# zju-pi/diff-sampler

Measured on AMD Instinct MI355X. Metric: images/sec (whole node) at NFE=10, EDM CIFAR-10, higher is better.
Workload: dtype fp32; 1 GPU; EDM CIFAR-10 32x32 SongUNet (55.7M params), DPM-Solver++(2M) logSNR NFE=10, batch 256/GPU; launch=eager

## Files before the change

diff_sampler_amd/csrc/conv3x3_wino.hip:

```cpp
#include <type_traits>

#include "igemm_common.h"

namespace igemm {
namespace {

typedef float f32x2 __attribute__((ext_vector_type(2)));

constexpr int WV_NO_NORM = 2, WV_NO_HALO = 4, WV_NO_DMA = 8, WV_NO_EPI = 16;
constexpr int WINO_K = 8;
constexpr int WINO_POS = 2 * 64 * 4;
constexpr int WINO_IMG = 16 * WINO_POS;
constexpr int WINO_NSH = 4;
constexpr int WINO_EPI_LD = 36;

#define DS_WINO_WAIT_VM0() do { __builtin_amdgcn_s_waitcnt(0x0F70); asm volatile("" ::: "memory"); } while (0)
#define DS_WINO_WAIT_VM(n) do { __builtin_amdgcn_s_waitcnt(0x0F70 | (n)); asm volatile("" ::: "memory"); } while (0)

template <int VAR, int NORM, int NSL>
__global__ void __launch_bounds__(256, 1) conv3x3_wino_kernel(const KParams p) {
    extern __shared__ __attribute__((aligned(16))) float smem[];
    float* Us = smem;
    float* Vs = smem + 2 * WINO_IMG;
    float* Hs = smem + 4 * WINO_IMG;
// ... 566 lines not shown
    };

    f32x16 acc[16];
#pragma unroll
    for (int q = 0; q < 16; ++q)
#pragma unroll
        for (int r = 0; r < 16; ++r) acc[q][r] = 0.f;
    const int a_off = ((lane >> 5) * 32 + (lane & 31)) * 4;

#define DS_WINO_I(n) std::integral_constant<int, (n)>{}
#define DS_WINO_EACH4(F) F(0) F(1) F(2) F(3)
#define DS_WINO_EACH12(F) F(0) F(1) F(2) F(3) F(4) F(5) F(6) F(7) F(8) F(9) F(10) F(11)
#define DS_WINO_EACH16(F, b) F((b) + 0) F((b) + 1) F((b) + 2) F((b) + 3) F((b) + 4) F((b) + 5) F((b) + 6) F((b) + 7)                \
                             F((b) + 8) F((b) + 9) F((b) + 10) F((b) + 11) F((b) + 12) F((b) + 13) F((b) + 14) F((b) + 15)
#define DS_WINO_LOADS(R, sl)                                                                                                           \
    halo_load1(R, DS_WINO_I(0)); halo_load1(R, DS_WINO_I(1)); halo_load1(R, DS_WINO_I(2));                                             \
    coef_load1(R, sl, DS_WINO_I(0)); coef_load1(R, sl, DS_WINO_I(1)); coef_load1(R, sl, DS_WINO_I(2));

    halo_src(0);
    DS_WINO_LOADS(hreg, 0)
    {
        HaloRegs hreg1;
        const int s1 = min(1, nslabs - 1);
        halo_src(s1);
        DS_WINO_LOADS(hreg1, s1)
#define DS_WINO_F(i) b_load1(u_src, DS_WINO_I(0), DS_WINO_I(i));
        DS_WINO_EACH4(DS_WINO_F)
#undef DS_WINO_F
        DS_RACE_SKEW(wave);
#define DS_WINO_CHAIN1(c) halo_chain(hreg, Hs, DS_WINO_I(c), DS_WINO_I(0)); halo_chain(hreg, Hs, DS_WINO_I(c), DS_WINO_I(1));          \
                          halo_chain(hreg, Hs, DS_WINO_I(c), DS_WINO_I(2));
        DS_WINO_EACH12(DS_WINO_CHAIN1)
#undef DS_WINO_CHAIN1
        DS_RACE_SKEW(wave);
#define DS_WINO_CHAIN1(c) halo_chain(hreg1, Hs + h_buf, DS_WINO_I(c), DS_WINO_I(0)); halo_chain(hreg1, Hs + h_buf, DS_WINO_I(c), DS_WINO_I(1)); \
                          halo_chain(hreg1, Hs + h_buf, DS_WINO_I(c), DS_WINO_I(2));
        DS_WINO_EACH12(DS_WINO_CHAIN1)
#undef DS_WINO_CHAIN1
    }
    {
        const int s2 = min(2, nslabs - 1);
        halo_src(s2);
        DS_WINO_LOADS(hreg, s2)
    }
    __syncthreads();
#define DS_WINO_TR1(i) tr_read1(Hs, DS_WINO_I(i));
    DS_WINO_EACH12(DS_WINO_TR1)
#undef DS_WINO_TR1
    DS_RACE_SKEW(wave);
    tr_write(Vs);
    DS_WINO_WAIT_VM0();
    __syncthreads();

    int s = 0;
    do {
        const int par = s & 1;
        const float* vb = Vs + par * WN_IMG;
        float* vbn = Vs + (par ^ 1) * WN_IMG;
        float* hb = Hs + par * h_buf;
        const float* hbn = Hs + (par ^ 1) * h_buf;
        const int s1 = min(s + 1, nslabs - 1), s3 = min(s + 3, nslabs - 1);
        const float* uc = u_src + (size_t)s * WINO_IMG;
        const float* un = u_src + (size_t)s1 * WINO_IMG;
        auto a_read = [&](auto G, auto I) {
            constexpr int g = decltype(G)::value, i = decltype(I)::value;
            fa[g & 1][i] = *reinterpret_cast<const f32x4*>(vb + (g * 4 + i) * WN_POS + a_off);
        };
#define DS_WINO_TR1(i) tr_read1(hbn, DS_WINO_I(i));
        DS_WINO_EACH12(DS_WINO_TR1)
#undef DS_WINO_TR1
        DS_RACE_SKEW(wave);
#define DS_WINO_CHAIN1(c) halo_chain(hreg, hb, DS_WINO_I(c), DS_WINO_I(0)); halo_chain(hreg, hb, DS_WINO_I(c), DS_WINO_I(1));          \
                          halo_chain(hreg, hb, DS_WINO_I(c), DS_WINO_I(2));
        DS_WINO_EACH12(DS_WINO_CHAIN1)
#undef DS_WINO_CHAIN1
        halo_src(s3);
        DS_RACE_SKEW(wave);
        tr_write(vbn);
        auto fill = [&](auto K) {
            constexpr int k = decltype(K)::value, g = k >> 4, q = k & 15;
            if constexpr (q < 4) {
                if constexpr (g < 3) b_load1(uc, DS_WINO_I(g + 1), DS_WINO_I(q));
                else b_load1(un, DS_WINO_I(0), DS_WINO_I(q));
            } else if constexpr (k < 7) {
                halo_load1(hreg, DS_WINO_I(k - 4));
            } else if constexpr (k < 10) {
                coef_load1(hreg, s3, DS_WINO_I(k - 7));
            } else if constexpr (q >= 10 && q < 14 && g < 3) {
                a_read(DS_WINO_I(g + 1), DS_WINO_I(q - 10));
            }
        };
#define DS_WINO_STEP(k)                                                                                                                \
        acc[((k) >> 4) * 4 + ((k) & 3)] = __builtin_amdgcn_mfma_f32_32x32x2f32(fa[((k) >> 4) & 1][(k) & 3][((k) >> 2) & 3],            \
                                                                               fb[((k) >> 4) & 1][(k) & 3][((k) >> 2) & 3],            \
                                                                               acc[((k) >> 4) * 4 + ((k) & 3)], 0, 0, 0);              \
        fill(DS_WINO_I(k));                                                                                                            \
        __builtin_amdgcn_sched_barrier(0);
#define DS_WINO_F(i) a_read(DS_WINO_I(0), DS_WINO_I(i));
        DS_WINO_EACH4(DS_WINO_F)
#undef DS_WINO_F
        __builtin_amdgcn_sched_barrier(0);
        DS_WINO_EACH16(DS_WINO_STEP, 0)
        DS_WINO_EACH16(DS_WINO_STEP, 16)
        DS_WINO_EACH16(DS_WINO_STEP, 32)
        DS_WINO_EACH16(DS_WINO_STEP, 48)
#undef DS_WINO_STEP
        __syncthreads();
    } while (++s < nslabs);
#undef DS_WINO_LOADS

    f32x16 Y[4];
#pragma unroll
    for (int a = 0; a < 2; ++a) {
        f32x16 t[4];
#pragma unroll
        for (int j = 0; j < 4; ++j) t[j] = a == 0 ? acc[j] + acc[4 + j] + acc[8 + j] : acc[4 + j] - acc[8 + j] - acc[12 + j];
        Y[a * 2 + 0] = t[0] + t[1] + t[2];
        Y[a * 2 + 1] = t[1] - t[2] - t[3];
    }

    const int nextra = (p.ec0 + p.ec1) / 32;
    if (nextra > 0) {
        const float* wsk = p.b + (size_t)(p.N / 64) * nslabs * WINO_IMG + (size_t)(2 * nt + (wave >> 1)) * nextra * 2048;
        const int e_chunk = tid & 7;
        int e_lds[4];
#pragma unroll
        for (int j = 0; j < 4; ++j) {
            const int lp = (tid >> 3) + 32 * j;
            const int yl = lp / p.W, x = lp - yl * p.W;
            const int ph = (yl & 1) * 2 + (x & 1), t = (yl >> 1) * Wt + (x >> 1);
            e_lds[j] = (((ph * 4 + (e_chunk >> 1)) * 2 + (e_chunk & 1)) * 32 + (t ^ e_chunk)) * 4;
        }
        int ea_off[4];
#pragma unroll
        for (int g = 0; g < 4; ++g) ea_off[g] = ((lane >> 5) * 32 + ((lane & 31) ^ (2 * g + (lane >> 5)))) * 4;
        const unsigned e_t0 = (unsigned)((tid >> 3) * p.elda0 + e_chunk * 4), e_t1 = (unsigned)((tid >> 3) * p.elda1 + e_chunk * 4);
        const float* e_src = nullptr;
        unsigned e_off = 0;
        int e_step = 0;
        auto e_sel = [&](int es) {
            const int c = es * 32;
            const bool first = c < p.ec0;
            const int ld = first ? p.elda0 : p.elda1;
            e_src = (first ? p.e0 + c : p.e1 + (c - p.ec0)) + (size_t)m0 * ld;
            e_step = 32 * ld;
            e_off = first ? e_t0 : e_t1;
        };
        auto e_load1 = [&](f32x4* dst, auto J) {
            constexpr int j = decltype(J)::value;
            dst[j] = *reinterpret_cast<const f32x4*>(e_src + (size_t)(j * e_step) + e_off);
        };
        f32x4 ga[2][4], gb[2];
        auto w_load1 = [&](int es, auto G) {
            constexpr int g = decltype(G)::value;
            const char* ws = reinterpret_cast<const char*>(wsk + (size_t)es * 2048 + g * WINO_POS);
            asm volatile("" : "+s"(ws));
            asm volatile("" : "+v"(b_lane));
            gb[g & 1] = *(gf4_t)(ws + b_lane);
        };

        f32x4 ereg[4];
        {
            f32x4 ereg0[4];
            w_load1(0, DS_WINO_I(0));
            e_sel(0);
#define DS_WINO_F(j) e_load1(ereg0, DS_WINO_I(j));
            DS_WINO_EACH4(DS_WINO_F)
#undef DS_WINO_F
            e_sel(min(1, nextra - 1));
#define DS_WINO_F(j) e_load1(ereg, DS_WINO_I(j));
            DS_WINO_EACH4(DS_WINO_F)
#undef DS_WINO_F
            DS_RACE_SKEW(wave);
#pragma unroll
            for (int j = 0; j < 4; ++j) *reinterpret_cast<f32x4*>(Vs + e_lds[j]) = ereg0[j];
        }
        __syncthreads();

        int es = 0;
        do {
            const float* vb = smem + (es & 1) * WN_IMG;
            float* vn = smem + ((es + 1) & 1) * WN_IMG;
            const int es1 = min(es + 1, nextra - 1);
            e_sel(min(es + 2, nextra - 1));
            auto a_read = [&](auto G, auto I) {
                constexpr int g = decltype(G)::value, i = decltype(I)::value;
                ga[g & 1][i] = *reinterpret_cast<const f32x4*>(vb + (i * 4 + g) * WN_POS + ea_off[g]);
            };
            auto fill = [&](auto K) {
                constexpr int k = decltype(K)::value, g = k >> 4, q = k & 15;
                if constexpr (q == 0) {
                    if constexpr (g < 3) w_load1(es, DS_WINO_I(g + 1));
                    else w_load1(es1, DS_WINO_I(0));
                } else if constexpr (q < 5) {
                    if constexpr (g < 3) a_read(DS_WINO_I(g + 1), DS_WINO_I(q - 1));
                } else if constexpr (k < 9) {
                    if constexpr (k == 5) DS_RACE_SKEW(wave);
                    *reinterpret_cast<f32x4*>(vn + e_lds[k - 5]) = ereg[k - 5];
                } else if constexpr (k < 13) {
                    e_load1(ereg, DS_WINO_I(k - 9));
                }
            };
#define DS_WINO_STEP(k)                                                                                                                \
            Y[(k) & 3] = __builtin_amdgcn_mfma_f32_32x32x2f32(ga[((k) >> 4) & 1][(k) & 3][((k) >> 2) & 3], gb[((k) >> 4) & 1][((k) >> 2) & 3], \
                                                              Y[(k) & 3], 0, 0, 0);                                                    \
            fill(DS_WINO_I(k));                                                                                                        \
            __builtin_amdgcn_sched_barrier(0);
#define DS_WINO_F(i) a_read(DS_WINO_I(0), DS_WINO_I(i));
            DS_WINO_EACH4(DS_WINO_F)
#undef DS_WINO_F
            __builtin_amdgcn_sched_barrier(0);
            DS_WINO_EACH16(DS_WINO_STEP, 0)
            DS_WINO_EACH16(DS_WINO_STEP, 16)
            DS_WINO_EACH16(DS_WINO_STEP, 32)
            DS_WINO_EACH16(DS_WINO_STEP, 48)
#undef DS_WINO_STEP
            __syncthreads();
        } while (++es < nextra);
    }
#undef DS_WINO_EACH16
#undef DS_WINO_EACH12
#undef DS_WINO_EACH4
#undef DS_WINO_I

    float* stage = smem + wave * 32 * WINO_EPI_LD;
    const int c4 = (lane & 7) * 4;
    const int col = n0 + wave * 32 + c4;
    f32x4 cb = {0.f, 0.f, 0.f, 0.f}, cvu = {0.f, 0.f, 0.f, 0.f};
    if (p.colbias) cb = *reinterpret_cast<const f32x4*>(p.colbias + col);
    if (p.cbias) cvu = *reinterpret_cast<const f32x4*>(p.cbias + (size_t)(p.cbias_bcast ? 0 : img0) * p.cbias_ld + col);
    const float acc_scale = __builtin_bit_cast(float, __builtin_amdgcn_readfirstlane(__builtin_bit_cast(int, p.acc_scale)));
    const float scale = __builtin_bit_cast(float, __builtin_amdgcn_readfirstlane(__builtin_bit_cast(int, p.scale)));
    int e_row[4];
#pragma unroll
    for (int pass = 0; pass < 4; ++pass) {
        const int tl = pass * 8 + (lane >> 3);
        const int ty = tl / Wt, tx = tl - ty * Wt;
        e_row[pass] = m0 + 2 * ty * p.W + 2 * tx;
    }
#pragma unroll
    for (int a = 0; a < 2; ++a) {
        f32x4 st_s = {0.f, 0.f, 0.f, 0.f}, st_q = {0.f, 0.f, 0.f, 0.f};
#pragma unroll
        for (int b = 0; b < 2; ++b) {
            const f32x16 y = Y[a * 2 + b];
            f32x4 rv[4];
            if (p.res) {
#pragma unroll
                for (int pass = 0; pass < 4; ++pass)
                    rv[pass] = __builtin_nontemporal_load(reinterpret_cast<const f32x4*>(p.res + (size_t)(e_row[pass] + a * p.W + b) * p.res_ld + col));
            }
#pragma unroll
            for (int r = 0; r < 16; ++r) stage[((r & 3) + 8 * (r >> 2) + 4 * (lane >> 5)) * WINO_EPI_LD + (lane & 31)] = y[r];
#pragma unroll
            for (int pass = 0; pass < 4; ++pass) {
                f32x4 v = *reinterpret_cast<const f32x4*>(stage + (pass * 8 + (lane >> 3)) * WINO_EPI_LD + c4);
                v *= acc_scale;
                v += cb;
                if (p.cbias) v += cvu;
                if (p.res) v += rv[pass];
                v *= scale;
                if (p.act == DS_ACT_SILU) {
#pragma unroll
                    for (int q = 0; q < 4; ++q) v[q] = ds_silu(v[q]);
                }
                __builtin_nontemporal_store(v, reinterpret_cast<f32x4*>(p.out + (size_t)(e_row[pass] + a * p.W + b) * p.ldo + col));
                st_s += v; st_q += v * v;
            }
        }
        if (p.stats) {
#pragma unroll
            for (int q = 0; q < 4; ++q) {
                st_s[q] += __shfl_xor(st_s[q], 8); st_s[q] += __shfl_xor(st_s[q], 16); st_s[q] += __shfl_xor(st_s[q], 32);
                st_q[q] += __shfl_xor(st_q[q], 8); st_q[q] += __shfl_xor(st_q[q], 16); st_q[q] += __shfl_xor(st_q[q], 32);
            }
            if (lane < 8) {
                float* sp = p.stats + (size_t)((m0 >> 6) + a) * 2 * p.N + col;
                *reinterpret_cast<f32x4*>(sp) = st_s;
                *reinterpret_cast<f32x4*>(sp + p.N) = st_q;
            }
        }
    }
}

template <int NORM, int NSL>
int launch_wino_n128_ns(KParams& p, hipStream_t stream) {
    const int smem = (2 * WN_IMG + 2 * (p.NP * WINO_K + 4)) * (int)sizeof(float);
    DS_ENSURE_DYN_LDS((&wino_n128_kernel<NORM, NSL>), 64 * 1024);
    hipLaunchKernelGGL((wino_n128_kernel<NORM, NSL>), dim3(grid_1d(p.mtiles, p.ntiles)), dim3(256), smem, stream, p);
    DS_CHECK_LAUNCH();
    return DS_OK;
}

template <int NORM>
int launch_wino_n128_n(KParams& p, hipStream_t stream) {
    return p.NP * 2 <= 2 * 256 ? launch_wino_n128_ns<NORM, 2>(p, stream) : launch_wino_n128_ns<NORM, 3>(p, stream);
}

int launch_wino_n128(KParams& p, hipStream_t stream) {
    if (!p.norm) return launch_wino_n128_n<0>(p, stream);
    return p.norm_act == DS_ACT_SILU ? launch_wino_n128_n<2>(p, stream) : launch_wino_n128_n<1>(p, stream);
}


template <int VAR, int NORM, int NSL>
int launch_wino_ns(KParams& p, hipStream_t stream) {
    const int smem = (4 * WINO_IMG + 2 * (p.NP * WINO_K + 4)) * (int)sizeof(float);
    DS_ENSURE_DYN_LDS((&conv3x3_wino_kernel<VAR, NORM, NSL>), 160 * 1024);
    hipLaunchKernelGGL((conv3x3_wino_kernel<VAR, NORM, NSL>), dim3(grid_1d(p.mtiles, p.ntiles)), dim3(256), smem, stream, p);
    DS_CHECK_LAUNCH();
    return DS_OK;
}

template <int VAR, int NORM>
int launch_wino_n(KParams& p, hipStream_t stream) {
    return p.NP * 2 <= 3 * 256 ? launch_wino_ns<VAR, NORM, 3>(p, stream) : launch_wino_ns<VAR, NORM, 4>(p, stream);
}

template <int VAR>
int launch_wino(KParams& p, hipStream_t stream) {
    if (!p.norm) return launch_wino_n<VAR, 0>(p, stream);
    return p.norm_act == DS_ACT_SILU ? launch_wino_n<VAR, 2>(p, stream) : launch_wino_n<VAR, 1>(p, stream);
}

}

bool conv3x3_wino_applicable(const KParams& p) {
    if (p.taps != 9 || p.stride != 1 || p.splits != 1 || (p.ec0 & 31) || (p.ec1 & 31)) return false;
    if ((p.H & 1) || (p.W & 1) || p.W < 4 || p.W > 64 || p.HW % 256 || 256 % p.W || ((256 / p.W) & 1)) return false;
    if ((p.N & 63) || (p.c0 % WINO_K) || (p.c1 % WINO_K) || !p.vec_ok || p.out_planar || p.out_f16 || p.res_f16 || p.rowbias) return false;
    if (p.act != DS_ACT_NONE && p.act != DS_ACT_SILU) return false;
    const int np = (256 / p.W + 2) * (p.W + 2);
    if (np * 2 > WINO_NSH * 256 || (4 * WINO_IMG + 2 * (np * WINO_K + 4)) * (int)sizeof(float) > 160 * 1024) return false;
    return p.M % 256 == 0;
}

int launch_conv3x3_wino(KParams& p, hipStream_t stream) {
    if (!conv3x3_wino_applicable(p)) return DS_E_SHAPE;
    p.TH = 256 / p.W; p.nimg = 1; p.HP = p.TH + 2; p.WP = p.W + 2; p.NP = p.HP * p.WP;
    p.mtiles = p.M / 256; p.ntiles = p.N / 64; p.n_begin = 0;
#ifdef DS_CONV_ABLATIONS
    if (p.t_variant & 0x10000) {
        switch (p.t_variant & 31) {
            case 2: return launch_wino<2>(p, stream);
            case 4: return launch_wino<4>(p, stream);
            case 8: return launch_wino<8>(p, stream);
            case 16: return launch_wino<16>(p, stream);
            case 28: return launch_wino<28>(p, stream);
            default: break;
        }
    }
#endif
    if (!(p.t_variant & 1024) && p.N % 128 == 0) {
        p.TH = 128 / p.W; p.HP = p.TH + 2; p.NP = p.HP * p.WP;
        p.mtiles = p.M / 128; p.ntiles = p.N / 128;
        return launch_wino_n128(p, stream);
    }
    return launch_wino<0>(p, stream);
}

}
```

Measured before the change: 494.0 images/sec.

## Add 8-wave Winograd conv3x3 kernel splitting output tile phases across waves

Adds a 512-thread Winograd conv3x3 kernel for the 128x128 tile path on widths 16 and 32. Eight waves split the work into two output-row phases of four channel groups each, and the partial transform results are combined through an LDS exchange before the epilogue. The main loop interleaves halo loads, norm coefficient loads and the input transform with the MFMA steps. The aim is more waves per tile to hide latency, at the cost of extra LDS traffic, higher register pressure and an added reduction step.

```diff
diff --git a/diff_sampler_amd/csrc/conv3x3_wino.hip b/diff_sampler_amd/csrc/conv3x3_wino.hip
--- a/diff_sampler_amd/csrc/conv3x3_wino.hip
+++ b/diff_sampler_amd/csrc/conv3x3_wino.hip
@@ -892,6 +892,450 @@
     return p.norm_act == DS_ACT_SILU ? launch_wino_n128_n<2>(p, stream) : launch_wino_n128_n<1>(p, stream);
 }
 
+constexpr int W8_NSH = 1;
+constexpr int W8_XCH = 4 * 16 * 64;
+
+template <int NORM>
+__global__ void __launch_bounds__(512, 1) wino_w8_kernel(const KParams p) {
+    extern __shared__ __attribute__((aligned(16))) float smem[];
+    float* Vs = smem;
+    float* Hs = smem + 2 * WN_IMG;
+
+    const int tid = threadIdx.x, lane = tid & 63;
+    const int wave = __builtin_amdgcn_readfirstlane(tid >> 6);
+    const int cg = wave & 3, ph = wave >> 2;
+    int mt, nt;
+    if (!decode_tile(blockIdx.x, p.mtiles, p.ntiles, mt, nt)) return;
+    const int m0 = mt * 128, n0 = nt * 128;
+    const int img0 = m0 / p.HW;
+    const int r0 = (m0 - img0 * p.HW) / p.W;
+    const int WPH = p.WP >> 1, Wt = p.W >> 1;
+    const int Ctot = p.c0 + p.c1;
+    const int nslabs = Ctot / WINO_K;
+
+    const int kh_h = tid & 1;
+    const int h_buf = p.NP * WINO_K + 4;
+    unsigned h_off0[W8_NSH], h_off1[W8_NSH];
+    int h_lds[W8_NSH];
+#pragma unroll
+    for (int j = 0; j < W8_NSH; ++j) {
+        const int hp = (tid + j * 512) >> 1;
+        const int hr = hp / p.WP, hc = hp - hr * p.WP;
+        const int y = r0 + hr - 1, x = hc - 1;
+        const bool in = hp < p.NP;
+        const bool ok = in && (unsigned)y < (unsigned)p.H && (unsigned)x < (unsigned)p.W;
+        const int pix = min(max(y, 0), p.H - 1) * p.W + min(max(x, 0), p.W - 1);
+        h_off0[j] = (unsigned)(pix * p.lda0 + kh_h * 4) * 4u;
+        h_off1[j] = (unsigned)(pix * p.lda1 + kh_h * 4) * 4u;
+        const int cell = (((kh_h * 2 + (hc & 1)) * p.HP + hr) * WPH + (hc >> 1)) * 4;
+        h_lds[j] = ok ? cell : p.NP * WINO_K;
+        if (in && !ok) {
+            const f32x4 z = {0.f, 0.f, 0.f, 0.f};
+            *reinterpret_cast<f32x4*>(Hs + cell) = z;
+            *reinterpret_cast<f32x4*>(Hs + h_buf + cell) = z;
+        }
+    }
+    const float* a0i = p.a0 + (size_t)img0 * p.HW * p.lda0;
+    const float* a1i = p.a1 + (size_t)img0 * p.HW * p.lda1;
+    const float* cpi = p.norm + (size_t)img0 * 3 * Ctot;
+    unsigned c_lane = (unsigned)(kh_h * 16);
+    struct HaloRegs {
+        f32x4 h[W8_NSH];
+        f32x4 mu = {0.f, 0.f, 0.f, 0.f}, ga = {1.f, 1.f, 1.f, 1.f}, be = {0.f, 0.f, 0.f, 0.f};
+    };
+    HaloRegs hreg;
+    float h_t[4 * W8_NSH], h_u[4 * W8_NSH];
+    const float* h_src = nullptr;
+    unsigned h_sel = 0;
+    auto halo_src = [&](int s) {
+        const int c = s * WINO_K;
+        const bool first = c < p.c0;
+        h_src = first ? a0i + c : a1i + (c - p.c0);
+        h_sel = (unsigned)__builtin_amdgcn_readfirstlane(first ? -1 : 0);
+        asm volatile("" : "+s"(h_sel));
+    };
+    auto halo_load1 = [&](HaloRegs& R, auto J) {
+        constexpr int j = decltype(J)::value;
+        if constexpr (j < W8_NSH) {
+            const unsigned off = (h_off0[j] & h_sel) | (h_off1[j] & ~h_sel);
+            R.h[j] = *reinterpret_cast<const f32x4*>(reinterpret_cast<const char*>(h_src) + off);
+        }
+    };
+    auto coef_load1 = [&](HaloRegs& R, int s, auto I) {
+        constexpr int i = decltype(I)::value;
+        if constexpr (NORM != 0) {
+            const char* cs = reinterpret_cast<const char*>(cpi + (size_t)i * Ctot + s * WINO_K);
+            asm volatile("" : "+v"(c_lane));
+            const f32x4 v = *reinterpret_cast<const f32x4*>(cs + c_lane);
+            if constexpr (i == 0) R.mu = v; else if constexpr (i == 1) R.ga = v; else R.be = v;
+        }
+    };
+    auto halo_chain = [&](HaloRegs& R, float* hs, auto C, auto ST) {
+        constexpr int c = decltype(C)::value, st = decltype(ST)::value, j = c >> 2, e = c & 3;
+        if constexpr (j < W8_NSH) {
+            if constexpr (st == 0 && NORM != 0) {
+                h_t[c] = __builtin_fmaf(R.h[j][e] - R.mu[e], R.ga[e], R.be[e]);
+                if constexpr (NORM == 2) h_u[c] = __expf(-h_t[c]);
+            }
+            if constexpr (st == 1 && NORM == 2) h_u[c] = __builtin_amdgcn_rcpf(1.0f + h_u[c]);
+            if constexpr (st == 2) {
+                float v = R.h[j][e];
+                if constexpr (NORM == 1) v = h_t[c];
+                if constexpr (NORM == 2) v = h_t[c] * h_u[c];
+                R.h[j][e] = v;
+                if constexpr (e == 3) *reinterpret_cast<f32x4*>(hs + h_lds[j]) = R.h[j];
+            }
+        }
+    };
+
+    const int t_t = (tid >> 1) & 31, cpl = tid & 1, kh_t = wave & 1, t_row = wave >> 1;
+    const int t_ty = t_t / Wt, t_tx = t_t - t_ty * Wt;
+    const int h_rd0 = ((kh_t * 2 * p.HP + 2 * t_ty + (t_row == 0 ? 0 : 1)) * WPH + t_tx) * 4 + cpl * 2;
+    const int h_rd1 = ((kh_t * 2 * p.HP + 2 * t_ty + (t_row == 3 ? 3 : 2)) * WPH + t_tx) * 4 + cpl * 2;
+    const int h_par = p.HP * WPH * 4;
+    const int v_wr = (kh_t * 32 + t_t) * 4 + cpl * 2 + t_row * 4 * WN_POS;
+    f32x2 t_e[2][4];
+    auto tr_read1 = [&](const float* hs, auto I) {
+        constexpr int i = decltype(I)::value >> 2, j = decltype(I)::value & 3;
+        t_e[i][j] = *reinterpret_cast<const f32x2*>(hs + (i == 0 ? h_rd0 : h_rd1) + (j & 1) * h_par + (j >> 1) * 4);
+    };
+    auto tr_write = [&](float* vs) {
+        f32x2 t_r[4];
+        if (t_row == 1) {
+#pragma unroll
+            for (int q = 0; q < 4; ++q) t_r[q] = t_e[0][q] + t_e[1][q];
+        } else if (t_row == 2) {
+#pragma unroll
+            for (int q = 0; q < 4; ++q) t_r[q] = t_e[1][q] - t_e[0][q];
+        } else {
+#pragma unroll
+            for (int q = 0; q < 4; ++q) t_r[q] = t_e[0][q] - t_e[1][q];
+        }
+#pragma unroll
+        for (int j = 0; j < 4; ++j) {
+            const f32x2 v = j == 0 ? t_r[0] - t_r[2] : j == 1 ? t_r[1] + t_r[2] : j == 2 ? t_r[2] - t_r[1] : t_r[1] - t_r[3];
+            *reinterpret_cast<f32x2*>(vs + v_wr + j * WN_POS) = v;
+        }
+    };
+
+    const float* u_src = p.b + (size_t)(2 * nt + (cg >> 1)) * nslabs * WINO_IMG + ph * 8 * WINO_POS;
+    unsigned b_lane = (unsigned)(((lane >> 5) * 64 + (cg & 1) * 32 + (lane & 31)) * 16);
+    f32x4 fa[2][4], fb[2][4];
+    typedef const __attribute__((address_space(1))) f32x4* gf4_t;
+    auto b_load1 = [&](const float* src, auto G, auto I) {
+        constexpr int g = decltype(G)::value, i = decltype(I)::value;
+        const char* us = reinterpret_cast<const char*>(src + (g * 4 + i) * WINO_POS);
+        asm volatile("" : "+s"(us));
+        asm volatile("" : "+v"(b_lane));
+        fb[g & 1][i] = *(gf4_t)(us + b_lane);
+    };
+
+    f32x16 acc[8];
+#pragma unroll
+    for (int q = 0; q < 8; ++q)
+#pragma unroll
+        for (int r = 0; r < 16; ++r) acc[q][r] = 0.f;
+    const int a_off = ((lane >> 5) * 32 + (lane & 31)) * 4 + ph * 8 * WN_POS;
+
+#define DS_WINO_I(n) std::integral_constant<int, (n)>{}
+#define DS_WINO_EACH4(F) F(0) F(1) F(2) F(3)
+#define DS_WINO_EACH8(F) F(0) F(1) F(2) F(3) F(4) F(5) F(6) F(7)
+#define DS_WINO_EACH16(F, b) F((b) + 0) F((b) + 1) F((b) + 2) F((b) + 3) F((b) + 4) F((b) + 5) F((b) + 6) F((b) + 7)                \
+                             F((b) + 8) F((b) + 9) F((b) + 10) F((b) + 11) F((b) + 12) F((b) + 13) F((b) + 14) F((b) + 15)
+#define DS_WINO_LOADS(R, sl)                                                                                                           \
+    halo_load1(R, DS_WINO_I(0));                                                                                                       \
+    coef_load1(R, sl, DS_WINO_I(0)); coef_load1(R, sl, DS_WINO_I(1)); coef_load1(R, sl, DS_WINO_I(2));
+
+    halo_src(0);
+    DS_WINO_LOADS(hreg, 0)
+    {
+        HaloRegs hreg1;
+        const int s1 = min(1, nslabs - 1);
+        halo_src(s1);
+        DS_WINO_LOADS(hreg1, s1)
+#define DS_WINO_F(i) b_load1(u_src, DS_WINO_I(0), DS_WINO_I(i));
+        DS_WINO_EACH4(DS_WINO_F)
+#undef DS_WINO_F
+        DS_RACE_SKEW(wave);
+#define DS_WINO_CHAIN1(c) halo_chain(hreg, Hs, DS_WINO_I(c), DS_WINO_I(0)); halo_chain(hreg, Hs, DS_WINO_I(c), DS_WINO_I(1));          \
+                          halo_chain(hreg, Hs, DS_WINO_I(c), DS_WINO_I(2));
+        DS_WINO_EACH4(DS_WINO_CHAIN1)
+#undef DS_WINO_CHAIN1
+        DS_RACE_SKEW(wave);
+#define DS_WINO_CHAIN1(c) halo_chain(hreg1, Hs + h_buf, DS_WINO_I(c), DS_WINO_I(0)); halo_chain(hreg1, Hs + h_buf, DS_WINO_I(c), DS_WINO_I(1)); \
+                          halo_chain(hreg1, Hs + h_buf, DS_WINO_I(c), DS_WINO_I(2));
+        DS_WINO_EACH4(DS_WINO_CHAIN1)
+#undef DS_WINO_CHAIN1
+    }
+    {
+        const int s2 = min(2, nslabs - 1);
+        halo_src(s2);
+        DS_WINO_LOADS(hreg, s2)
+    }
+    __syncthreads();
+#define DS_WINO_TR1(i) tr_read1(Hs, DS_WINO_I(i));
+    DS_WINO_EACH8(DS_WINO_TR1)
+#undef DS_WINO_TR1
+    DS_RACE_SKEW(wave);
+    tr_write(Vs);
+    DS_WINO_WAIT_VM0();
+    __syncthreads();
+
+    int s = 0;
+    do {
+        const int par = s & 1;
+        const float* vb = Vs + par * WN_IMG;
+        float* vbn = Vs + (par ^ 1) * WN_IMG;
+        float* hb = Hs + par * h_buf;
+        const float* hbn = Hs + (par ^ 1) * h_buf;
+        const int s1 = min(s + 1, nslabs - 1), s3 = min(s + 3, nslabs - 1);
+        const float* uc = u_src + (size_t)s * WINO_IMG;
+        const float* un = u_src + (size_t)s1 * WINO_IMG;
+        auto a_read = [&](auto G, auto I) {
+            constexpr int g = decltype(G)::value, i = decltype(I)::value;
+            fa[g & 1][i] = *reinterpret_cast<const f32x4*>(vb + (g * 4 + i) * WN_POS + a_off);
+        };
+#define DS_WINO_TR1(i) tr_read1(hbn, DS_WINO_I(i));
+        DS_WINO_EACH8(DS_WINO_TR1)
+#undef DS_WINO_TR1
+        DS_RACE_SKEW(wave);
+#define DS_WINO_CHAIN1(c) halo_chain(hreg, hb, DS_WINO_I(c), DS_WINO_I(0)); halo_chain(hreg, hb, DS_WINO_I(c), DS_WINO_I(1));          \
+                          halo_chain(hreg, hb, DS_WINO_I(c), DS_WINO_I(2));
+        DS_WINO_EACH4(DS_WINO_CHAIN1)
+#undef DS_WINO_CHAIN1
+        halo_src(s3);
+        DS_RACE_SKEW(wave);
+        tr_write(vbn);
+        auto fill = [&](auto K) {
+            constexpr int k = decltype(K)::value, g = k >> 4, q = k & 15;
+            if constexpr (q < 4) {
+                if constexpr (g == 0) b_load1(uc, DS_WINO_I(1), DS_WINO_I(q));
+                else b_load1(un, DS_WINO_I(0), DS_WINO_I(q));
+            } else if constexpr (k == 4) {
+                halo_load1(hreg, DS_WINO_I(0));
+            } else if constexpr (k < 8) {
+                coef_load1(hreg, s3, DS_WINO_I(k - 5));
+            } else if constexpr (k >= 10 && k < 14) {
+                a_read(DS_WINO_I(1), DS_WINO_I(k - 10));
+            }
+        };
+#define DS_WINO_STEP(k)                                                                                                                \
+        acc[((k) >> 4) * 4 + ((k) & 3)] = __builtin_amdgcn_mfma_f32_32x32x2f32(fa[((k) >> 4) & 1][(k) & 3][((k) >> 2) & 3],            \
+                                                                               fb[((k) >> 4) & 1][(k) & 3][((k) >> 2) & 3],            \
+                                                                               acc[((k) >> 4) * 4 + ((k) & 3)], 0, 0, 0);              \
+        fill(DS_WINO_I(k));                                                                                                            \
+        __builtin_amdgcn_sched_barrier(0);
+#define DS_WINO_F(i) a_read(DS_WINO_I(0), DS_WINO_I(i));
+        DS_WINO_EACH4(DS_WINO_F)
+#undef DS_WINO_F
+        __builtin_amdgcn_sched_barrier(0);
+        DS_WINO_EACH16(DS_WINO_STEP, 0)
+        DS_WINO_EACH16(DS_WINO_STEP, 16)
+#undef DS_WINO_STEP
+        __syncthreads();
+    } while (++s < nslabs);
+#undef DS_WINO_LOADS
+
+    f32x16 Y[2];
+    {
+        float* xw = smem + wave * W8_XCH + lane * 4;
+        const float* xr = smem + (wave ^ 4) * W8_XCH + lane * 4;
+        DS_RACE_SKEW(wave);
+#pragma unroll
+        for (int q = 0; q < 4; ++q) {
+            const f32x16 m = ph == 0 ? acc[4 + q] : acc[q];
+#pragma unroll
+            for (int r4 = 0; r4 < 4; ++r4) {
+                const f32x4 v = {m[4 * r4], m[4 * r4 + 1], m[4 * r4 + 2], m[4 * r4 + 3]};
+                *reinterpret_cast<f32x4*>(xw + (q * 4 + r4) * 256) = v;
+            }
+        }
+        __syncthreads();
+        f32x16 t[4];
+#pragma unroll
+        for (int j = 0; j < 4; ++j) {
+            f32x16 o;
+#pragma unroll
+            for (int r4 = 0; r4 < 4; ++r4) {
+                const f32x4 v = *reinterpret_cast<const f32x4*>(xr + (j * 4 + r4) * 256);
+                o[4 * r4] = v[0]; o[4 * r4 + 1] = v[1]; o[4 * r4 + 2] = v[2]; o[4 * r4 + 3] = v[3];
+            }
+            if (ph == 0) t[j] = acc[j] + acc[4 + j] + o;
+            else t[j] = o - acc[j] - acc[4 + j];
+        }
+        Y[0] = t[0] + t[1] + t[2];
+        Y[1] = t[1] - t[2] - t[3];
+    }
+
+    const int nextra = (p.ec0 + p.ec1) / 32;
+    if (nextra > 0) {
+        __syncthreads();
+        const float* wsk = p.b + (size_t)(p.N / 64) * nslabs * WINO_IMG + (size_t)(2 * nt + (cg >> 1)) * nextra * 2048;
+        const int e_chunk = tid & 7;
+        int e_lds[2];
+#pragma unroll
+        for (int j = 0; j < 2; ++j) {
+            const int lp = (tid >> 3) + 64 * j;
+            const int yl = lp / p.W, x = lp - yl * p.W;
+            const int pp = (yl & 1) * 2 + (x & 1), t = (yl >> 1) * Wt + (x >> 1);
+            e_lds[j] = (((pp * 4 + (e_chunk >> 1)) * 2 + (e_chunk & 1)) * 32 + (t ^ e_chunk)) * 4;
+        }
+        int ea_off[4];
+#pragma unroll
+        for (int g = 0; g < 4; ++g) ea_off[g] = ((lane >> 5) * 32 + ((lane & 31) ^ (2 * g + (lane >> 5)))) * 4;
+        const unsigned e_t0 = (unsigned)((tid >> 3) * p.elda0 + e_chunk * 4), e_t1 = (unsigned)((tid >> 3) * p.elda1 + e_chunk * 4);
+        const float* e_src = nullptr;
+        unsigned e_off = 0;
+        int e_step = 0;
+        auto e_sel = [&](int es) {
+            const int c = es * 32;
+            const bool first = c < p.ec0;
+            const int ld = first ? p.elda0 : p.elda1;
+            e_src = (first ? p.e0 + c : p.e1 + (c - p.ec0)) + (size_t)m0 * ld;
+            e_step = 64 * ld;
+            e_off = first ? e_t0 : e_t1;
+        };
+        auto e_load1 = [&](f32x4* dst, auto J) {
+            constexpr int j = decltype(J)::value;
+            dst[j] = *reinterpret_cast<const f32x4*>(e_src + (size_t)(j * e_step) + e_off);
+        };
+        f32x4 ga[2][2], gb[4];
+        auto w_load1 = [&](int es, auto G) {
+            constexpr int g = decltype(G)::value;
+            const char* ws = reinterpret_cast<const char*>(wsk + (size_t)es * 2048 + g * WINO_POS);
+            asm volatile("" : "+s"(ws));
+            asm volatile("" : "+v"(b_lane));
+            gb[g] = *(gf4_t)(ws + b_lane);
+        };
+
+        f32x4 ereg[2];
+        {
+            f32x4 ereg0[2];
+            w_load1(0, DS_WINO_I(0)); w_load1(0, DS_WINO_I(1)); w_load1(0, DS_WINO_I(2)); w_load1(0, DS_WINO_I(3));
+            e_sel(0);
+            e_load1(ereg0, DS_WINO_I(0)); e_load1(ereg0, DS_WINO_I(1));
+            e_sel(min(1, nextra - 1));
+            e_load1(ereg, DS_WINO_I(0)); e_load1(ereg, DS_WINO_I(1));
+            DS_RACE_SKEW(wave);
+#pragma unroll
+            for (int j = 0; j < 2; ++j) *reinterpret_cast<f32x4*>(Vs + e_lds[j]) = ereg0[j];
+        }
+        __syncthreads();
+
+        int es = 0;
+        do {
+            const float* vb = smem + (es & 1) * WN_IMG + ph * 8 * WN_POS;
+            float* vn = smem + ((es + 1) & 1) * WN_IMG;
+            const int es1 = min(es + 1, nextra - 1);
+            e_sel(min(es + 2, nextra - 1));
+            auto a_read = [&](auto G, auto I) {
+                constexpr int g = decltype(G)::value, i = decltype(I)::value;
+                ga[g & 1][i] = *reinterpret_cast<const f32x4*>(vb + (i * 4 + g) * WN_POS + ea_off[g]);
+            };
+            auto fill = [&](auto K) {
+                constexpr int k = decltype(K)::value, g = k >> 3, q = k & 7;
+                if constexpr (q == 0) {
+                    if constexpr (g >= 1) w_load1(es1, DS_WINO_I(g - 1));
+                } else if constexpr (q < 3) {
+                    if constexpr (g < 3) a_read(DS_WINO_I(g + 1), DS_WINO_I(q - 1));
+                } else if constexpr (k < 5) {
+                    if constexpr (k == 3) DS_RACE_SKEW(wave);
+                    *reinterpret_cast<f32x4*>(vn + e_lds[k - 3]) = ereg[k - 3];
+                } else if constexpr (k < 7) {
+                    e_load1(ereg, DS_WINO_I(k - 5));
+                } else if constexpr (k == 31) {
+                    w_load1(es1, DS_WINO_I(3));
+                }
+            };
+#define DS_WINO_STEP(k)                                                                                                                \
+            Y[(k) & 1] = __builtin_amdgcn_mfma_f32_32x32x2f32(ga[((k) >> 3) & 1][(k) & 1][((k) >> 1) & 3], gb[(k) >> 3][((k) >> 1) & 3], \
+                                                              Y[(k) & 1], 0, 0, 0);                                                    \
+            fill(DS_WINO_I(k));                                                                                                        \
+            __builtin_amdgcn_sched_barrier(0);
+            a_read(DS_WINO_I(0), DS_WINO_I(0)); a_read(DS_WINO_I(0), DS_WINO_I(1));
+            __builtin_amdgcn_sched_barrier(0);
+            DS_WINO_EACH16(DS_WINO_STEP, 0)
+            DS_WINO_EACH16(DS_WINO_STEP, 16)
+#undef DS_WINO_STEP
+            __syncthreads();
+        } while (++es < nextra);
+    }
+#undef DS_WINO_EACH16
+#undef DS_WINO_EACH8
+#undef DS_WINO_EACH4
+#undef DS_WINO_I
+
+    float* stage = smem + (wave ^ 4) * W8_XCH;
+    const int c4 = (lane & 7) * 4;
+    const int col = n0 + cg * 32 + c4;
+    f32x4 cb = {0.f, 0.f, 0.f, 0.f}, cvu = {0.f, 0.f, 0.f, 0.f};
+    if (p.colbias) cb = *reinterpret_cast<const f32x4*>(p.colbias + col);
+    if (p.cbias) cvu = *reinterpret_cast<const f32x4*>(p.cbias + (size_t)(p.cbias_bcast ? 0 : img0) * p.cbias_ld + col);
+    const float acc_scale = __builtin_bit_cast(float, __builtin_amdgcn_readfirstlane(__builtin_bit_cast(int, p.acc_scale)));
+    const float scale = __builtin_bit_cast(float, __builtin_amdgcn_readfirstlane(__builtin_bit_cast(int, p.scale)));
+    int e_row[4];
+#pragma unroll
+    for (int pass = 0; pass < 4; ++pass) {
+        const int tl = pass * 8 + (lane >> 3);
+        const int ty = tl / Wt, tx = tl - ty * Wt;
+        e_row[pass] = m0 + (2 * ty + ph) * p.W + 2 * tx;
+    }
+    f32x4 st_s = {0.f, 0.f, 0.f, 0.f}, st_q = {0.f, 0.f, 0.f, 0.f};
+#pragma unroll
+    for (int b = 0; b < 2; ++b) {
+        const f32x16 y = Y[b];
+        f32x4 rv[4];
+        if (p.res) {
+#pragma unroll
+            for (int pass = 0; pass < 4; ++pass)
+                rv[pass] = __builtin_nontemporal_load(reinterpret_cast<const f32x4*>(p.res + (size_t)(e_row[pass] + b) * p.res_ld + col));
+        }
+#pragma unroll
+        for (int r = 0; r < 16; ++r) stage[((r & 3) + 8 * (r >> 2) + 4 * (lane >> 5)) * WINO_EPI_LD + (lane & 31)] = y[r];
+#pragma unroll
+        for (int pass = 0; pass < 4; ++pass) {
+            f32x4 v = *reinterpret_cast<const f32x4*>(stage + (pass * 8 + (lane >> 3)) * WINO_EPI_LD + c4);
+            v *= acc_scale;
+            v += cb;
+            if (p.cbias) v += cvu;
+            if (p.res) v += rv[pass];
+            v *= scale;
+            if (p.act == DS_ACT_SILU) {
+#pragma unroll
+                for (int q = 0; q < 4; ++q) v[q] = ds_silu(v[q]);
+            }
+            __builtin_nontemporal_store(v, reinterpret_cast<f32x4*>(p.out + (size_t)(e_row[pass] + b) * p.ldo + col));
+            st_s += v; st_q += v * v;
+        }
+    }
+    if (p.stats) {
+#pragma unroll
+        for (int q = 0; q < 4; ++q) {
+            st_s[q] += __shfl_xor(st_s[q], 8); st_s[q] += __shfl_xor(st_s[q], 16); st_s[q] += __shfl_xor(st_s[q], 32);
+            st_q[q] += __shfl_xor(st_q[q], 8); st_q[q] += __shfl_xor(st_q[q], 16); st_q[q] += __shfl_xor(st_q[q], 32);
+        }
+        if (lane < 8) {
+            float* sp = p.stats + (size_t)((m0 >> 6) + ph) * 2 * p.N + col;
+            *reinterpret_cast<f32x4*>(sp) = st_s;
+            *reinterpret_cast<f32x4*>(sp + p.N) = st_q;
+        }
+    }
+}
+
+template <int NORM>
+int launch_wino_w8_n(KParams& p, hipStream_t stream) {
+    const int kloop = (2 * WN_IMG + 2 * (p.NP * WINO_K + 4)) * (int)sizeof(float), xch = 8 * W8_XCH * (int)sizeof(float);
+    DS_ENSURE_DYN_LDS((&wino_w8_kernel<NORM>), 160 * 1024);
+    hipLaunchKernelGGL((wino_w8_kernel<NORM>), dim3(grid_1d(p.mtiles, p.ntiles)), dim3(512), kloop > xch ? kloop : xch, stream, p);
+    DS_CHECK_LAUNCH();
+    return DS_OK;
+}
+
+int launch_wino_w8(KParams& p, hipStream_t stream) {
+    if (!p.norm) return launch_wino_w8_n<0>(p, stream);
+    return p.norm_act == DS_ACT_SILU ? launch_wino_w8_n<2>(p, stream) : launch_wino_w8_n<1>(p, stream);
+}
+
 
 template <int VAR, int NORM, int NSL>
 int launch_wino_ns(KParams& p, hipStream_t stream) {
@@ -944,7 +1388,8 @@
     if (!(p.t_variant & 1024) && p.N % 128 == 0) {
         p.TH = 128 / p.W; p.HP = p.TH + 2; p.NP = p.HP * p.WP;
         p.mtiles = p.M / 128; p.ntiles = p.N / 128;
-        return launch_wino_n128(p, stream);
+        const bool w8 = (p.W == 16 || p.W == 32) && !(p.t_variant & 32768);
+        return w8 ? launch_wino_w8(p, stream) : launch_wino_n128(p, stream);
     }
     return launch_wino<0>(p, stream);
 }
```

After: 509.6 images/sec (median of 6 runs). 1.03x the previous value.
